# ieellee/uLLSAM

Hardware: AMD Instinct MI355X
Metric: images/s end-to-end (ViT+LLM+mask) 1024^2 (higher is better)
Workload: dtype bf16; 1 GPU; uLLSAM mask path (app.py:580-645): SAM ViT-H + InternLM2-7b-shaped prefill S=1081 + prompt encoder + mask decoder + x4 upsample/threshold, 1 point prompt/image, batch 4/GPU; batch_per_gpu=4, global_batch=4, seq_len=1081, vit_linears=bf16

## Files before the change

### include/ullsam_hip.h

```cpp
#ifndef ULLSAM_HIP_H
#define ULLSAM_HIP_H
#ifdef __cplusplus
extern "C" {
#endif

#define ULLSAM_DT_F32 0
#define ULLSAM_DT_BF16 1
#define ULLSAM_ACT_NONE 0
#define ULLSAM_ACT_GELU 1
#define ULLSAM_ACT_RELU 2
#define ULLSAM_ACT_SWIGLU 3

#define ULLSAM_ABI_VERSION 14

const char* ullsam_last_error_string(void);
int ullsam_abi_version(void);
int ullsam_device_count(void);
int ullsam_set_gemm_variant(int variant);
int ullsam_set_gemm_tuning(int key, int value);
int ullsam_set_attn_variant(int variant);
int ullsam_set_attn_debug(void* stamps);

#define ULLSAM_ACT_SPLITK_OK 256
int ullsam_gemm(int dtype, const void* A, long lda, const void* W, long ldw, void* C, long ldc, int out_f32,
// ... 64 lines not shown
                               void* table_grad, int out_dtype, void* stream);
int ullsam_train_index_add_rows(const float* src, const int* idx, float* dst, long rows, int C, int nrows_dst, void* stream);

int ullsam_norm(const void* in, int in_dtype, long in_stride, void* out, int out_dtype, long out_stride, const float* w,
                const float* b, long rows, int D, float eps, int rms, int act, const float* post_scale,
                const float* post_shift, void* stream);
int ullsam_norm_panels(const void* in, int in_dtype, long in_stride, void* out, const float* w, const float* b, long rows, int D, float eps, int rms,
                       int act, const float* post_scale, const float* post_shift, int out_panels, void* stream);
int ullsam_set_norm_variant(int v);

int ullsam_norm_fanout(const float* in, long rows, int D, const float* w, const float* b, float eps, float* out_f32, void* out_c,
                       void* out_c_pe, int c_dtype, const float* pe, long pe_rows, void* stream);

int ullsam_vit_attention(int dtype, const void* qkv, void* out, const void* rel_h, const void* rel_w, const void* qkv_bias,
                         int B, int heads, int hd, int grid_h, int grid_w, int window, void* stream);

int ullsam_causal_attention(int dtype, const void* q, const void* k, const void* v, void* out, const int* key_mask, int B,
                            int H, int KVH, int hd, int Sq, int Sk, int k_cap, int q_pos0, void* stream);

int ullsam_naive_attention(int dtype, const void* q, const void* k, const void* v, void* out, const int* key_mask, int B,
                           int H, int KVH, int hd, int Sq, int Sk, long q_bs, long q_ts, long q_hs, long k_bs, long k_ts,
                           long k_hs, long v_bs, long v_ts, long v_hs, long o_bs, long o_ts, long o_hs, float scale,
                           void* stream);

int ullsam_decode_attention(const void* q, const void* kc, const void* vc, const int* key_mask, void* out, int B, int H, int KVH,
                            int hd, int Sk, int cap, float scale, float* workspace, int nsplit, void* stream);

int ullsam_fewkeys_attention(const float* q, const float* k, const float* v, float* out, int B, int H, int hd, int Sq,
                             int Sk, float scale, long q_batch_stride, void* stream);

int ullsam_tok2img_attention(int kv_dtype, const float* q, const void* k, const void* v, float* out, int P, int H, int hd, int T,
                             int N, long k_batch_stride, long v_batch_stride, float scale, float* workspace, int nsplit,
                             void* stream);
// ... 223 lines not shown
```

### ullsam_amd/_lib.py

```python
from __future__ import annotations

import ctypes as C
import os

_HERE = os.path.dirname(os.path.abspath(__file__))
LIB_PATH = os.environ.get("ULLSAM_HIP_LIB") or os.path.join(_HERE, "lib", "libullsam_hip.so")

ABI_VERSION = 14

_lib = None

vp, i32, i64, f32 = C.c_void_p, C.c_int, C.c_long, C.c_float

SIGNATURES = {
    "ullsam_gemm": [i32, vp, i64, vp, i64, vp, i64, i32, vp, vp, i64, i32, i32, i32, i32, i32, vp, i64, vp],
    "ullsam_gemm_qkv_rope": [i32, vp, i64, vp, i64, vp, i32, i32, i32, i32, i32, vp, vp, vp, i32, vp, vp, vp, i32, i32, vp, i64, vp],
    "ullsam_gemm_panels": [i32, vp, i64, vp, i64, vp, vp, i64, i32, vp, vp, i64, i32, i32, i32, i32, i32, vp, i64, vp],
    "ullsam_gemm_qkv_rope_panels": [i32, vp, i64, vp, i64, vp, vp, i32, i32, i32, i32, i32, vp, vp, vp, i32, vp, vp, vp, i32, i32, vp, i64, vp],
    "ullsam_gemm_act_panels": [i32, vp, i64, vp, i64, vp, vp, i64, i32, vp, vp, i64, i32, i32, i32, i32, i32, vp, i64, i32, i32, vp],
    "ullsam_gemm_qkv_rope_act_panels": [i32, vp, i64, vp, i64, vp, vp, i32, i32, i32, i32, i32, vp, vp, vp, i32, vp, vp, vp, i32, i32, vp, i64, i32, vp],
    "ullsam_gemm_act_panels_query": [i32, i32, i32, i32, i32, i32, i32, i32, i32, i64, vp, vp],
    "ullsam_gemm_rmsnorm": [vp, i64, vp, f32, vp, i64, vp, i64, i32, vp, vp, i64, i32, i32, i32, i32, vp],
    "ullsam_decode_qkv_rope": [vp, vp, i64, vp, f32, vp, i64, vp, i32, i32, i32, i32, vp, vp, vp, i32, vp, vp, vp, i32, i32, vp],
    "ullsam_train_matmul": [vp, vp, vp, i32, i32, i32, i32] + [i64] * 9 + [i32, vp],
# ... 11 lines not shown
    "ullsam_train_rope": [vp, vp, vp, vp, vp, i64, i32, i32, i32, i32, vp],
    "ullsam_train_swiglu": [vp, vp, vp, vp, vp, vp, i64, vp],
    "ullsam_train_resize_bwd": [vp, vp, i64, i32, i32, i32, i32, vp],
    "ullsam_train_seg_loss": [vp, vp, vp, vp, i32, i64, f32, vp, vp],
    "ullsam_train_seg_loss_bwd": [vp, vp, vp, vp, vp, i32, i64, f32, vp],
    "ullsam_train_cross_entropy": [vp, i64, vp, vp, vp, vp, i64, i32, vp],
    "ullsam_train_cross_entropy_bwd": [vp, i64, vp, vp, vp, vp, vp, i64, i64, i32, vp],
    "ullsam_train_cross_entropy_bwd_bf16": [vp, i64, vp, vp, vp, vp, vp, i64, vp, i64, i64, i32, vp],
    "ullsam_train_embedding_bwd": [vp, i64, vp, vp, vp, i64, i32, i32, i32, vp, i32, vp],
    "ullsam_train_index_add_rows": [vp, vp, vp, i64, i32, i32, vp],
    "ullsam_norm": [vp, i32, i64, vp, i32, i64, vp, vp, i64, i32, f32, i32, i32, vp, vp, vp],
    "ullsam_norm_panels": [vp, i32, i64, vp, vp, vp, i64, i32, f32, i32, i32, vp, vp, i32, vp],
    "ullsam_norm_fanout": [vp, i64, i32, vp, vp, f32, vp, vp, vp, i32, vp, i64, vp],
    "ullsam_vit_attention": [i32, vp, vp, vp, vp, vp, i32, i32, i32, i32, i32, i32, vp],
    "ullsam_causal_attention": [i32, vp, vp, vp, vp, vp, i32, i32, i32, i32, i32, i32, i32, i32, vp],
    "ullsam_naive_attention": [i32, vp, vp, vp, vp, vp, i32, i32, i32, i32, i32, i32] + [i64] * 12 + [f32, vp],
    "ullsam_fewkeys_attention": [vp, vp, vp, vp, i32, i32, i32, i32, i32, f32, i64, vp],
    "ullsam_decode_attention": [vp, vp, vp, vp, vp, i32, i32, i32, i32, i32, i32, f32, vp, i32, vp],
    "ullsam_tok2img_attention": [i32, vp, vp, vp, vp, i32, i32, i32, i32, i32, i64, i64, f32, vp, i32, vp],
    "ullsam_patch_im2col": [i32, vp, vp, i32, i32, i32, i32, i32, i32, vp, vp, vp],
    "ullsam_im2col3x3": [i32, vp, vp, i32, i32, i32, i32, vp],
    "ullsam_add_cast": [vp, i32, i64, vp, i64, vp, i32, i64, i32, vp],
    "ullsam_transpose_f32": [vp, vp, i32, i32, i32, vp],
    "ullsam_transpose_to_bf16": [i32, vp, vp, i32, i32, i32, vp],
    "ullsam_cast_transpose_bf16": [vp, vp, vp, vp, vp, i32, i32, i32, vp],
    "ullsam_pixel_shuffle_ln": [i32, vp, vp, vp, vp, i32, i32, i32, i32, f32, vp],
    "ullsam_pixel_unshuffle": [vp, vp, i32, i32, i32, i32, vp],
    "ullsam_scan_image_tokens": [vp, vp, vp, i32, i32, C.c_longlong, vp],
    "ullsam_embed_tokens": [i32, vp, vp, vp, vp, vp, i32, i32, i32, i32, i64, vp],
    "ullsam_gather_rows": [vp, vp, vp, i32, i32, i32, i32, vp],
# ... 142 lines not shown
```

### ullsam_amd/csrc/attention.hip

```cpp
#include "common.h"
#include <type_traits>

enum { MODE_PLAIN = 0, MODE_CAUSAL = 1, MODE_VIT_GLOBAL = 2, MODE_VIT_WINDOW = 3 };

struct AttnArgs {
    const void* q; const void* k; const void* v; void* out;
    long q_bs, q_ts, q_hs;
    long k_bs, k_ts, k_hs;
    long v_bs, v_ts, v_hs;
    long o_bs, o_ts, o_hs;
    int B, H, groups;
    int Sq, Sk;
    float scale;
    const int* key_mask;
    int q_pos0;
    const void* rel_h; const void* rel_w;
    int grid_h, grid_w;
    int win, nwin_w, nwin;
    const void* bias_q; const void* bias_k; const void* bias_v;
    unsigned long long* dbg;
};

template <typename T, int HD, int TR = 64> struct KVTile {
    static constexpr int RS = HD * (int)sizeof(T) + 16;
    static constexpr int ROWS = TR;
    static constexpr int BYTES = RS * ROWS;
    static constexpr int CPR = HD * (int)sizeof(T) / 16;
    static constexpr int RSV = sizeof(T) == 2 ? 320 : RS;
    static constexpr int VBYTES = RSV * ROWS;
    static_assert(sizeof(T) != 2 || HD * 2 <= 256, "V row does not fit its 320-byte stride");
};

template <int RS>
__device__ __forceinline__ Frag<bf16> load_vt_frag(const char* vt, int kv0, int d0, int lane, const bf16*) {
    const int grp = lane >> 4, i = lane & 15;
    const int h = grp >> 1;
// ... 1002 lines not shown
            mma16(vf[m % NV], pf[m / 5], o[m % 5]);
            if (m % 5 == 4) mma16(ones, pf[m / 5], o[5]);
            __builtin_amdgcn_sched_barrier(0);
            if (m + NV < NVI) vf[m % NV] = vread(m + NV);
        }
        __builtin_amdgcn_sched_barrier(0);
        const float inv_l = 1.0f / o[5][0];
        char* ob = reinterpret_cast<char*>(scr);
#pragma unroll
        for (int d = 0; d < 5; ++d) {
            bf16x4_t v;
            v[0] = (bf16)(o[d][0] * inv_l); v[1] = (bf16)(o[d][1] * inv_l); v[2] = (bf16)(o[d][2] * inv_l); v[3] = (bf16)(o[d][3] * inv_l);
            *reinterpret_cast<bf16x4_t*>(ob + ql * 160 + 32 * d + 8 * g) = v;
        }
        asm volatile("" ::: "memory");
        T* orow = reinterpret_cast<T*>(p.out) + (long)b * p.o_bs + (long)head * p.o_hs;
        const int qgy = wy * G + cur_qh;
#pragma unroll
        for (int r = 0; r < 3; ++r) {
            const int c = lane + 64 * r;
            const int qq = c / 10, ch = c - 10 * qq;
            const int gx = wx * G + qq;
            if (c < 16 * 10 && qq < G && gx < p.grid_w) {
                const uint4 v = *reinterpret_cast<const uint4*>(ob + 16 * c);
                *reinterpret_cast<uint4*>(orow + ((long)qgy * p.grid_w + gx) * p.o_ts + 8 * ch) = v;
            }
        }
        asm volatile("" ::: "memory");
    };
    stamp(2);
    asm volatile("s_waitcnt vmcnt(0)" ::: "memory");
    stamp(3);
    __syncthreads();
    stamp(4);
    if (live[0]) main_group(0, qf0, cinit0, thr0);
    stamp(5);
    if (live[1]) main_group(1, qf1, cinit1, thr1);
    stamp(6);
}

// ... 241 lines not shown
        const unsigned long long s2 = STAMP ? __builtin_amdgcn_s_memtime() : 0ull;
        if (tile + 1 < ntiles && tid < TR) kms[((tile + 1) & 1) * TR + tid] = km_next;
        __syncthreads();
        if (STAMP) { const unsigned long long s3 = __builtin_amdgcn_s_memtime(); st_dma += s1 - s0; st_cmp += s2 - s1; st_bar += s3 - s2; }
    }
    if (STAMP && p.dbg && lane == 0) {
        unsigned long long* d = p.dbg + ((size_t)(blockIdx.y * gridDim.x + blockIdx.x) * 4 + wave) * 8;
        d[0] = st_dma; d[1] = st_cmp; d[2] = st_bar; d[3] = __builtin_amdgcn_s_memtime() - st_t0; d[4] = ntiles; d[5] = qblk;
        d[6] = st_r0; d[7] = __builtin_amdgcn_s_memrealtime();
    }

    float lo, hi;
    halves(l_run, lo, hi);
    const float l_tot = lo + hi;
    const float inv_l = l_tot > 0.f ? 1.0f / l_tot : 0.f;
    if (q_valid) {
        T* op = reinterpret_cast<T*>(p.out) + (long)b * p.o_bs + (long)qi * p.o_ts + (long)head * p.o_hs;
#pragma unroll
        for (int d = 0; d < DT; ++d)
#pragma unroll
            for (int rq = 0; rq < 4; ++rq)
                store4(op + 32 * d + 8 * rq + 4 * h, make_float4(o[d][4 * rq] * inv_l, o[d][4 * rq + 1] * inv_l, o[d][4 * rq + 2] * inv_l, o[d][4 * rq + 3] * inv_l));
    }
}

static int launch_causal128(const AttnArgs& a, hipStream_t s) {
    constexpr int LDS = 2 * 2 * 64 * 256 + 2 * 64 * 4;
    static PerDeviceOnce attr;
    if (attr.first()) {
        (void)hipFuncSetAttribute(reinterpret_cast<const void*>(causal128_attn_kernel<false>), hipFuncAttributeMaxDynamicSharedMemorySize, LDS);
        (void)hipFuncSetAttribute(reinterpret_cast<const void*>(causal128_attn_kernel<true>), hipFuncAttributeMaxDynamicSharedMemorySize, LDS);
    }
    if (a.dbg) causal128_attn_kernel<true><<<dim3(a.H * a.B, (a.Sq + 127) / 128), dim3(256), LDS, s>>>(a);
    else causal128_attn_kernel<false><<<dim3(a.H * a.B, (a.Sq + 127) / 128), dim3(256), LDS, s>>>(a);
    ULLSAM_LAUNCH_CHECK();
    return 0;
}
// ... 239 lines not shown
        };
#pragma unroll 1
        for (int j = 0; j < NB; j += 4) {
            interval(j, I0{}, sc0, sc1);
            interval(j + 1, I1{}, sc1, sc0);
            interval(j + 2, I2{}, sc0, sc1);
            interval(j + 3, I3{}, sc1, sc0);
        }
    }
    asm volatile("s_waitcnt vmcnt(0)" ::: "memory");

    float lo, hi;
    halves(o[DT - 1][8], lo, hi);
    const float l_tot = lo;
    const float inv_l = l_tot > 0.f ? 1.0f / l_tot : 0.f;
    T* op = reinterpret_cast<T*>(p.out) + (long)b * p.o_bs + (long)qi * p.o_ts + (long)head * p.o_hs;
#pragma unroll
    for (int d = 0; d < DT; ++d)
#pragma unroll
        for (int rq = 0; rq < 4; ++rq) {
            const int dd = 32 * d + 8 * rq + 4 * h;
            if (dd < HD) store4(op + dd, make_float4(o[d][4 * rq] * inv_l, o[d][4 * rq + 1] * inv_l, o[d][4 * rq + 2] * inv_l, o[d][4 * rq + 3] * inv_l));
        }
}

static int launch_vitglob(const AttnArgs& a, hipStream_t s) {
    constexpr int LDS = 8 * 32 * 256 + 128 * (80 * 2 + 16) + 8 * 64 * 32 * 4;
    static PerDeviceOnce attr;
    if (attr.first()) (void)hipFuncSetAttribute(reinterpret_cast<const void*>(vitglob_attn_kernel), hipFuncAttributeMaxDynamicSharedMemorySize, LDS);
    vitglob_attn_kernel<<<dim3(a.B * a.H * 16), dim3(512), LDS, s>>>(a);
    ULLSAM_LAUNCH_CHECK();
    return 0;
}

static int g_attn_variant = 0;
static unsigned long long* g_attn_dbg = nullptr;
extern "C" int ullsam_set_attn_variant(int v) { g_attn_variant = v; return 0; }
extern "C" int ullsam_set_attn_debug(void* stamps) { g_attn_dbg = reinterpret_cast<unsigned long long*>(stamps); return 0; }

extern "C" int ullsam_vit_attention(int dtype, const void* qkv, void* out, const void* rel_h, const void* rel_w,
                                    const void* qkv_bias, int B, int heads, int hd, int grid_h, int grid_w, int window,
                                    void* stream) {
    ULLSAM_CHECK(dtype == 0 || dtype == 1, "vit_attention: bad dtype");
    ULLSAM_CHECK(grid_h <= 64 && grid_w <= 64 && window <= 14, "vit_attention: grid %dx%d / window %d too large", grid_h, grid_w, window);
    const int esz = dtype == 0 ? 4 : 2;
    ULLSAM_CHECK((hd * esz) % 16 == 0, "vit_attention: head_dim*elem must be a multiple of 16 bytes");
    ULLSAM_CHECK((((uintptr_t)qkv | (uintptr_t)out | (uintptr_t)qkv_bias | (uintptr_t)rel_h | (uintptr_t)rel_w) & 15) == 0,
                 "vit_attention: qkv, out, rel_h, rel_w and qkv_bias must be 16-byte aligned");
    const long D = (long)heads * hd;
    const long N = (long)grid_h * grid_w;
    AttnArgs a = {};
    const char* base = reinterpret_cast<const char*>(qkv);
    a.q = base; a.k = base + D * esz; a.v = base + 2 * D * esz; a.out = out;
    a.q_bs = a.k_bs = a.v_bs = N * 3 * D; a.q_ts = a.k_ts = a.v_ts = 3 * D; a.q_hs = a.k_hs = a.v_hs = hd;
    a.o_bs = N * D; a.o_ts = D; a.o_hs = hd;
    a.B = B; a.H = heads; a.groups = 1;
    a.scale = 1.0f / sqrtf((float)hd);
    a.rel_h = rel_h; a.rel_w = rel_w; a.grid_h = grid_h; a.grid_w = grid_w;
    const char* bb = reinterpret_cast<const char*>(qkv_bias);
    a.bias_q = bb; a.bias_k = bb + D * esz; a.bias_v = bb + 2 * D * esz;
    hipStream_t s = reinterpret_cast<hipStream_t>(stream);
    if (window > 0) {
        a.win = window;
        a.nwin_w = (grid_w + window - 1) / window;
        a.nwin = a.nwin_w * ((grid_h + window - 1) / window);
        a.Sq = a.Sk = window * window;
        a.q_pos0 = (g_attn_variant >= 3 && g_attn_variant <= 8) ? g_attn_variant - 3 : 2;
        if (dtype == 1 && window == 14 && hd == 80 && g_attn_variant != 1 && g_attn_variant != 2 && g_attn_variant != 13) {
            a.q_pos0 = (g_attn_variant >= 3 && g_attn_variant <= 8) ? g_attn_variant - 3 : 0;
            a.dbg = g_attn_dbg;
            return launch_win14r(a, s);
        }
        if (dtype == 1 && window == 14 && hd == 80 && g_attn_variant != 1 && g_attn_variant != 2) return launch_win14(a, s);
        if (g_attn_variant == 1) return dtype == 0 ? dispatch_hd<float, MODE_VIT_WINDOW, 7>(a, hd, s) : dispatch_hd<bf16, MODE_VIT_WINDOW, 7>(a, hd, s);
        return dtype == 0 ? dispatch_hd<float, MODE_VIT_WINDOW, 7>(a, hd, s) : dispatch_hd<bf16, MODE_VIT_WINDOW, 4>(a, hd, s);
    }
    a.Sq = a.Sk = (int)N;
    if (dtype == 1 && grid_h == 64 && grid_w == 64 && hd == 80 && g_attn_variant != 9 && g_attn_variant != 12)
        return launch_vitglob(a, s);
    if (dtype == 1 && grid_h == 64 && grid_w == 64 && g_attn_variant != 9) return dispatch_hd<bf16, MODE_VIT_GLOBAL, 8>(a, hd, s);
    return dtype == 0 ? dispatch_hd<float, MODE_VIT_GLOBAL, 4>(a, hd, s) : dispatch_hd<bf16, MODE_VIT_GLOBAL, 4>(a, hd, s);
}

extern "C" int ullsam_causal_attention(int dtype, const void* q, const void* k, const void* v, void* out, const int* key_mask,
                                       int B, int H, int KVH, int hd, int Sq, int Sk, int k_cap, int q_pos0, void* stream) {
    ULLSAM_CHECK(dtype == 0 || dtype == 1, "causal_attention: bad dtype");
    ULLSAM_CHECK(H % KVH == 0, "causal_attention: H %% KVH != 0");
    ULLSAM_CHECK((((uintptr_t)q | (uintptr_t)k | (uintptr_t)v | (uintptr_t)out) & 15) == 0, "causal_attention: q, k, v and out must be 16-byte aligned");
    AttnArgs a = {};
    a.q = q; a.k = k; a.v = v; a.out = out;
    a.q_bs = (long)Sq * H * hd; a.q_ts = (long)H * hd; a.q_hs = hd;
    a.k_bs = a.v_bs = (long)KVH * k_cap * hd; a.k_ts = a.v_ts = hd; a.k_hs = a.v_hs = (long)k_cap * hd;
    a.o_bs = a.q_bs; a.o_ts = a.q_ts; a.o_hs = hd;
    a.B = B; a.H = H; a.groups = H / KVH; a.Sq = Sq; a.Sk = Sk; a.key_mask = key_mask; a.q_pos0 = q_pos0;
    a.scale = 1.0f / sqrtf((float)hd);
    a.dbg = g_attn_dbg;
    hipStream_t s = reinterpret_cast<hipStream_t>(stream);
    if (dtype == 1 && hd == 128 && g_attn_variant != 11 && a.k_ts == 128 && a.v_ts == 128)
        return launch_causal128(a, s);
    return dtype == 0 ? dispatch_hd<float, MODE_CAUSAL, 4>(a, hd, s) : dispatch_hd<bf16, MODE_CAUSAL, 4>(a, hd, s);
}

struct NaiveArgs {
    const void* q; const void* k; const void* v; void* out;
    long q_bs, q_ts, q_hs, k_bs, k_ts, k_hs, v_bs, v_ts, v_hs, o_bs, o_ts, o_hs;
    int H, groups, Sq, Sk, hd;
    float scale;
    const int* key_mask;
};

template <typename T>
__global__ __launch_bounds__(256) void naive_attn_kernel(NaiveArgs p) {
    extern __shared__ __attribute__((aligned(16))) char smem[];
    float* sc = reinterpret_cast<float*>(smem);
    float* qs = sc + ((p.Sk + 3) & ~3);
// ... 634 lines not shown
```

### ullsam_amd/modeling/image_encoder.py

```python
from __future__ import annotations

from typing import Optional, Tuple, Type

import torch
from torch import nn

from .. import ops
from ..packing import pack_conv3x3
from .common import LayerNorm, LayerNorm2d, Linear, MLPBlock, Packed


class _Conv2dParams(Packed):

    def __init__(self, cin, cout, k, bias=True):
        super().__init__()
        self.weight = nn.Parameter(torch.empty(cout, cin, k, k))
        self.bias = nn.Parameter(torch.zeros(cout)) if bias else None
        nn.init.normal_(self.weight, std=(cin * k * k) ** -0.5)


class PatchEmbed(Packed):

    def __init__(self, kernel_size=(16, 16), stride=(16, 16), padding=(0, 0), in_chans=3, embed_dim=768):
        super().__init__()
# ... 94 lines not shown
        pos = None if self.pos_embed is None else self.f32("pos", self.pos_embed).reshape(N, D)
        xres = ops.gemm(cols, wp, None if pe.bias is None else self.f32("patch_b", pe.bias), residual=pos, res_row_mod=N, out_f32=True)
        fp8 = bool(self.fp8_linears) and dt == torch.bfloat16 and D % 128 == 0
        M, hp = xres.shape[0], False
        for bi, blk in enumerate(self.blocks):
            at = blk.attn
            if fp8:
                q8, sa = ops.rows_fp8(xres, *blk.norm1.wb(), blk.norm1.eps)
                qkv = ops.gemm_fp8(q8, sa, *at.qkv.w8(), at.qkv.b())
            else:
                ap, _ = ops.activation_panels_plan(M, 3 * D, D, dt, bias=at.qkv.b() is not None)
                xn = ops.norm(xres, *blk.norm1.wb(), blk.norm1.eps, dt, out_panels=ap)
                qkv = ops.gemm(xn, at.qkv.w(dt), at.qkv.b(), w_panels=at.qkv.wp(dt, M), a_panels=ap, m=M)
            qb = at.qkv.bias if at.qkv.bias is not None else torch.zeros(3 * D, device=x.device)
            n_rel = blk.window_size if blk.window_size > 0 else g
            att = ops.vit_attention(qkv, at.rel_table("rh", at.rel_pos_h, n_rel, dt), at.rel_table("rw", at.rel_pos_w, n_rel, dt), at.cdt("qb", qb, dt),
                                    B, self.num_heads, at.head_dim, g, g, blk.window_size)
            ops.gemm(att, at.proj.w(dt), at.proj.b(), residual=xres, out_f32=True, out=xres, w_panels=at.proj.wp(dt, att.shape[0]))
            if fp8:
                q8, sa = ops.rows_fp8(xres, *blk.norm2.wb(), blk.norm2.eps)
                h = ops.gemm_fp8(q8, sa, *blk.mlp.lin1.w8(), blk.mlp.lin1.b(), act=blk.mlp.act_code)
            else:
                w1, w2 = blk.mlp.lin1.w(dt), blk.mlp.lin2.w(dt)
                ap, cp = ops.activation_panels_plan(M, w1.shape[0], D, dt, act=blk.mlp.act_code, bias=blk.mlp.lin1.b() is not None)
                hp = cp and ops.activation_panels_plan(M, D, w2.shape[1], dt, out_f32=True, bias=blk.mlp.lin2.b() is not None, residual=True)[0]
                xn = ops.norm(xres, *blk.norm2.wb(), blk.norm2.eps, dt, out_panels=ap)
                h = ops.gemm(xn, w1, blk.mlp.lin1.b(), act=blk.mlp.act_code, w_panels=blk.mlp.lin1.wp(dt, M), a_panels=ap, out_panels=hp, m=M)
            ops.gemm(h, blk.mlp.lin2.w(dt), blk.mlp.lin2.b(), residual=xres, out_f32=True, out=xres, w_panels=blk.mlp.lin2.wp(dt, M), a_panels=hp, m=M)
            if self.stage_probe is not None:
                self.stage_probe(bi, xres)
        n0, n1, n2, n3 = self.neck[0], self.neck[1], self.neck[2], self.neck[3]
        C = self.out_chans
        w0 = self.pk("neck0", n0.weight, lambda: n0.weight.detach().reshape(C, D).to(dt).contiguous())
# ... 17 lines not shown
```

### ullsam_amd/modeling/modeling_internlm2.py

```python
from __future__ import annotations

from typing import List, Optional, Tuple

import torch
from torch import nn

from .. import ops
from ..packing import pack_w13
from ..sampling import row_seeds
from .common import Linear, Packed, ring_panels
from .configuration_internlm2 import InternLM2Config
from .outputs import BaseModelOutputWithPast, CausalLMOutputWithPast


class InternLM2RMSNorm(Packed):

    def __init__(self, hidden_size, eps=1e-6):
        super().__init__()
        self.weight = nn.Parameter(torch.ones(hidden_size))
        self.variance_epsilon = eps

    def w(self):
        return self.f32("w", self.weight)

# ... 154 lines not shown
            if w8:
                q = ops.decode_qkv_rope_w8(x, layer.attention_norm.w(), layer.attention_norm.variance_epsilon, *at.wqkv.w8d(), at.wqkv.b(), kc, vc,
                                           pos, cos, sin, B, KVH, G, past)
            elif fused:
                q = ops.decode_qkv_rope(x, layer.attention_norm.w(), layer.attention_norm.variance_epsilon, at.wqkv.w(dt), at.wqkv.b(), kc, vc,
                                        pos, cos, sin, B, KVH, G, past)
            else:
                wq, rope_ep = at.wqkv.w(dt), hd == 128 and S > 8
                ap, _ = ops.activation_panels_plan(B * S, wq.shape[0], wq.shape[1], dt, bias=at.wqkv.b() is not None, rope=rope_ep)
                xn = ops.norm(x, layer.attention_norm.w(), None, layer.attention_norm.variance_epsilon, dt, rms=True, out_panels=ap)
                if rope_ep:
                    q = ops.gemm_qkv_rope(xn, wq, at.wqkv.b(), kc, vc, pos, cos, sin, B, S, KVH, G, past, w_panels=at.wqkv.wp(dt, B * S), a_panels=ap)
                else:
                    qkv = ops.gemm(xn, wq, at.wqkv.b(), w_panels=at.wqkv.wp(dt, B * S), a_panels=ap, m=B * S)
                    q = ops.rope_split(qkv, kc, vc, pos, cos, sin, B, S, KVH, G, hd, past)
            if S > 1:
                a = ops.causal_attention(q, kc, vc, key_mask, B, H, KVH, hd, S, Sk, past)
            elif dt == torch.bfloat16 and hd == 128 and G <= 8:
                a = ops.decode_attention(q, kc, vc, key_mask, B, H, KVH, hd, Sk)
            else:
                cap = kc.shape[2]
                a = ops.naive_attention(q, kc, vc, B, H, KVH, hd, 1, Sk, (H * hd, H * hd, hd), (KVH * cap * hd, hd, cap * hd),
                                        (KVH * cap * hd, hd, cap * hd), (H * hd, H * hd, hd), hd ** -0.5, key_mask=key_mask)
            if w8_wo:
                ops.gemm_w8(a, *at.wo.w8d(), at.wo.b(), residual=x, out_f32=True, out=x)
            else:
                ops.gemm(a, at.wo.w(dt), at.wo.b(), residual=x, out_f32=True, out=x, w_panels=at.wo.wp(dt, B * S))
            if w8:
                hmid = ops.gemm_w8(x, *ff.w13_w8d(dt), act=ops.ACT_SWIGLU, norm_w=layer.ffn_norm.w(), eps=layer.ffn_norm.variance_epsilon)
            elif fused:
                hmid = ops.gemm_rmsnorm(x, layer.ffn_norm.w(), layer.ffn_norm.variance_epsilon, ff.w13(dt), act=ops.ACT_SWIGLU)
            else:
                w13, w2 = ff.w13(dt), ff.w2.w(dt)
                ap, cp = ops.activation_panels_plan(B * S, w13.shape[0], w13.shape[1], dt, act=ops.ACT_SWIGLU)
                hp = cp and not w8_w2 and ops.activation_panels_plan(B * S, w2.shape[0], w2.shape[1], dt, out_f32=True, residual=True)[0]
                xn = ops.norm(x, layer.ffn_norm.w(), None, layer.ffn_norm.variance_epsilon, dt, rms=True, out_panels=ap)
                hmid = ops.gemm(xn, w13, act=ops.ACT_SWIGLU, w_panels=ff.w13p(dt, B * S), a_panels=ap, out_panels=hp, m=B * S)
            if w8_w2:
                ops.gemm_w8(hmid, *ff.w2.w8d(), None, residual=x, out_f32=True, out=x)
            else:
                ops.gemm(hmid, ff.w2.w(dt), None, residual=x, out_f32=True, out=x, w_panels=ff.w2.wp(dt, B * S), a_panels=hp, m=B * S)
            if self.stage_probe is not None:
# ... 204 lines not shown
```

### ullsam_amd/ops.py

```python
from __future__ import annotations

import os
from typing import Optional

import numpy as np
import torch

from . import _lib

ACT_NONE, ACT_GELU, ACT_RELU, ACT_SWIGLU = 0, 1, 2, 3
ACT_SPLITK_OK = 256
_DT = {torch.float32: 0, torch.bfloat16: 1}


def dt_code(dtype: torch.dtype) -> int:
    try:
        return _DT[dtype]
    except KeyError:
        raise TypeError(f"ullsam_amd supports float32 and bfloat16 compute, got {dtype}") from None


def _stream() -> int:
    return torch.cuda.current_stream().cuda_stream

# ... 260 lines not shown
    _chk(hs, "hs", torch.float32)
    hyper = torch.empty((P, nm, 32), dtype=torch.float32, device=hs.device)
    iou = torch.empty((P, n_iou), dtype=torch.float32, device=hs.device)
    _lib.call("ullsam_dec_heads", hs.data_ptr(), w_ptrs.data_ptr(), b_ptrs.data_ptr(), hyper.data_ptr(), iou.data_ptr(), P, T, n_iou, m0, nm, _stream())
    return hyper, iou


def concat_token_rows(prefix: torch.Tensor, rows: torch.Tensor) -> torch.Tensor:
    _chk(prefix, "prefix", torch.float32); _chk(rows, "rows", torch.float32)
    P, n1, C = rows.shape
    out = torch.empty((P, prefix.shape[0] + n1, C), dtype=torch.float32, device=rows.device)
    _lib.call("ullsam_concat_token_rows", prefix.data_ptr(), prefix.shape[0], rows.data_ptr() if n1 else None, n1, out.data_ptr(), P, C, _stream())
    return out


def vit_attention(qkv: torch.Tensor, rel_h: torch.Tensor, rel_w: torch.Tensor, qkv_bias: torch.Tensor, B: int, heads: int,
                  hd: int, gh: int, gw: int, window: int) -> torch.Tensor:
    _chk(qkv, "qkv"); _chk(rel_h, "rel_h", qkv.dtype); _chk(rel_w, "rel_w", qkv.dtype); _chk(qkv_bias, "qkv_bias", qkv.dtype)
    D = heads * hd
    assert qkv.numel() == B * gh * gw * 3 * D
    n = window if window > 0 else gh
    assert rel_h.shape == (2 * n - 1, hd) and rel_w.shape[1] == hd
    out = torch.empty((B * gh * gw, D), dtype=qkv.dtype, device=qkv.device)
    _lib.call("ullsam_vit_attention", dt_code(qkv.dtype), qkv.data_ptr(), out.data_ptr(), rel_h.data_ptr(), rel_w.data_ptr(),
              qkv_bias.data_ptr(), B, heads, hd, gh, gw, window, _stream())
    return out


def causal_attention(q: torch.Tensor, k_cache: torch.Tensor, v_cache: torch.Tensor, key_mask: Optional[torch.Tensor],
                     B: int, H: int, KVH: int, hd: int, Sq: int, Sk: int, q_pos0: int) -> torch.Tensor:
    _chk(q, "q"); _chk(k_cache, "k_cache", q.dtype); _chk(v_cache, "v_cache", q.dtype)
    cap = k_cache.shape[2]
    if key_mask is not None:
        _chk(key_mask, "key_mask", torch.int32)
        assert key_mask.shape == (B, Sk)
    out = torch.empty((B * Sq, H * hd), dtype=q.dtype, device=q.device)
    _lib.call("ullsam_causal_attention", dt_code(q.dtype), q.data_ptr(), k_cache.data_ptr(), v_cache.data_ptr(), out.data_ptr(),
              _p(key_mask), B, H, KVH, hd, Sq, Sk, cap, q_pos0, _stream())
    return out


def naive_attention(q, k, v, B, H, KVH, hd, Sq, Sk, qs, ks, vs, os_, scale, key_mask=None, out=None):
    _chk(q, "q"); _chk(k, "k", q.dtype); _chk(v, "v", q.dtype)
    if out is None:
        out = torch.empty((B * Sq, H * hd), dtype=q.dtype, device=q.device)
    if key_mask is not None:
        _chk(key_mask, "key_mask", torch.int32)
    _lib.call("ullsam_naive_attention", dt_code(q.dtype), q.data_ptr(), k.data_ptr(), v.data_ptr(), out.data_ptr(), _p(key_mask),
              B, H, KVH, hd, Sq, Sk, *qs, *ks, *vs, *os_, float(scale), _stream())
    return out

# ... 1797 lines not shown
```

Baseline: 58.07 images/s.

## Write attention outputs directly in GEMM K-panel layout for output projections

The ViT windowed/global attention and the LLM causal prefill attention kernels can now stage their output tile in LDS and store it in the 16x32 K-panel layout that the following output-projection GEMM consumes as pre-paneled A. The proj/wo GEMMs are then called with a_panels set, so they skip their own repacking of the activation. Query entry points report whether the chosen kernel supports this, and an environment mask turns it on by default. The cost is extra LDS staging and swizzled scatter stores in the attention epilogues, plus a 1 KiB alignment requirement on the output buffer.

```diff
diff --git a/include/ullsam_hip.h b/include/ullsam_hip.h
--- a/include/ullsam_hip.h
+++ b/include/ullsam_hip.h
@@ -102,9 +102,15 @@
 
 int ullsam_vit_attention(int dtype, const void* qkv, void* out, const void* rel_h, const void* rel_w, const void* qkv_bias,
                          int B, int heads, int hd, int grid_h, int grid_w, int window, void* stream);
+int ullsam_vit_attention_out(int dtype, const void* qkv, void* out, const void* rel_h, const void* rel_w, const void* qkv_bias,
+                             int B, int heads, int hd, int grid_h, int grid_w, int window, int out_panels, void* stream);
+int ullsam_vit_attention_panels_query(int dtype, int heads, int hd, int grid_h, int grid_w, int window, int* writes_panels);
 
 int ullsam_causal_attention(int dtype, const void* q, const void* k, const void* v, void* out, const int* key_mask, int B,
                             int H, int KVH, int hd, int Sq, int Sk, int k_cap, int q_pos0, void* stream);
+int ullsam_causal_attention_out(int dtype, const void* q, const void* k, const void* v, void* out, const int* key_mask, int B,
+                                int H, int KVH, int hd, int Sq, int Sk, int k_cap, int q_pos0, int out_mode, void* stream);
+int ullsam_causal_attention_panels_query(int dtype, int H, int KVH, int hd, int* writes_panels);
 
 int ullsam_naive_attention(int dtype, const void* q, const void* k, const void* v, void* out, const int* key_mask, int B,
                            int H, int KVH, int hd, int Sq, int Sk, long q_bs, long q_ts, long q_hs, long k_bs, long k_ts,
diff --git a/ullsam_amd/_lib.py b/ullsam_amd/_lib.py
--- a/ullsam_amd/_lib.py
+++ b/ullsam_amd/_lib.py
@@ -49,6 +49,10 @@
     "ullsam_norm_fanout": [vp, i64, i32, vp, vp, f32, vp, vp, vp, i32, vp, i64, vp],
     "ullsam_vit_attention": [i32, vp, vp, vp, vp, vp, i32, i32, i32, i32, i32, i32, vp],
     "ullsam_causal_attention": [i32, vp, vp, vp, vp, vp, i32, i32, i32, i32, i32, i32, i32, i32, vp],
+    "ullsam_vit_attention_out": [i32, vp, vp, vp, vp, vp, i32, i32, i32, i32, i32, i32, i32, vp],
+    "ullsam_vit_attention_panels_query": [i32, i32, i32, i32, i32, i32, vp],
+    "ullsam_causal_attention_out": [i32, vp, vp, vp, vp, vp, i32, i32, i32, i32, i32, i32, i32, i32, i32, vp],
+    "ullsam_causal_attention_panels_query": [i32, i32, i32, i32, vp],
     "ullsam_naive_attention": [i32, vp, vp, vp, vp, vp, i32, i32, i32, i32, i32, i32] + [i64] * 12 + [f32, vp],
     "ullsam_fewkeys_attention": [vp, vp, vp, vp, i32, i32, i32, i32, i32, f32, i64, vp],
     "ullsam_decode_attention": [vp, vp, vp, vp, vp, i32, i32, i32, i32, i32, i32, f32, vp, i32, vp],
diff --git a/ullsam_amd/csrc/attention.hip b/ullsam_amd/csrc/attention.hip
--- a/ullsam_amd/csrc/attention.hip
+++ b/ullsam_amd/csrc/attention.hip
@@ -19,7 +19,13 @@
     int win, nwin_w, nwin;
     const void* bias_q; const void* bias_k; const void* bias_v;
     unsigned long long* dbg;
+    int out_mode;
 };
+enum { ATTN_OUT_ROWS = 0, ATTN_OUT_ROWS_STAGED = 1, ATTN_OUT_PANELS = 2 };
+
+__device__ __forceinline__ long panel_at(long row, int col, int K) {
+    return ((row >> 4) * (K >> 5) + (col >> 5)) * 512 + (row & 15) * 32 + (col & 31);
+}
 
 template <typename T, int HD, int TR = 64> struct KVTile {
     static constexpr int RS = HD * (int)sizeof(T) + 16;
@@ -1052,7 +1058,9 @@
             *reinterpret_cast<bf16x4_t*>(ob + ql * 160 + 32 * d + 8 * g) = v;
         }
         asm volatile("" ::: "memory");
-        T* orow = reinterpret_cast<T*>(p.out) + (long)b * p.o_bs + (long)head * p.o_hs;
+        const bool panels = p.out_mode == ATTN_OUT_PANELS;
+        T* orow = reinterpret_cast<T*>(p.out) + (panels ? 0 : (long)b * p.o_bs + (long)head * p.o_hs);
+        const long prow0 = (long)b * p.grid_h * p.grid_w;
         const int qgy = wy * G + cur_qh;
 #pragma unroll
         for (int r = 0; r < 3; ++r) {
@@ -1061,7 +1069,8 @@
             const int gx = wx * G + qq;
             if (c < 16 * 10 && qq < G && gx < p.grid_w) {
                 const uint4 v = *reinterpret_cast<const uint4*>(ob + 16 * c);
-                *reinterpret_cast<uint4*>(orow + ((long)qgy * p.grid_w + gx) * p.o_ts + 8 * ch) = v;
+                const long tok = (long)qgy * p.grid_w + gx;
+                *reinterpret_cast<uint4*>(orow + (panels ? panel_at(prow0 + tok, head * 80 + 8 * ch, (int)p.o_ts) : tok * p.o_ts + 8 * ch)) = v;
             }
         }
         asm volatile("" ::: "memory");
@@ -1333,13 +1342,40 @@
     halves(l_run, lo, hi);
     const float l_tot = lo + hi;
     const float inv_l = l_tot > 0.f ? 1.0f / l_tot : 0.f;
-    if (q_valid) {
-        T* op = reinterpret_cast<T*>(p.out) + (long)b * p.o_bs + (long)qi * p.o_ts + (long)head * p.o_hs;
-#pragma unroll
-        for (int d = 0; d < DT; ++d)
-#pragma unroll
-            for (int rq = 0; rq < 4; ++rq)
-                store4(op + 32 * d + 8 * rq + 4 * h, make_float4(o[d][4 * rq] * inv_l, o[d][4 * rq + 1] * inv_l, o[d][4 * rq + 2] * inv_l, o[d][4 * rq + 3] * inv_l));
+    if (p.out_mode == ATTN_OUT_ROWS) {
+        if (q_valid) {
+            T* op = reinterpret_cast<T*>(p.out) + (long)b * p.o_bs + (long)qi * p.o_ts + (long)head * p.o_hs;
+#pragma unroll
+            for (int d = 0; d < DT; ++d)
+#pragma unroll
+                for (int rq = 0; rq < 4; ++rq)
+                    store4(op + 32 * d + 8 * rq + 4 * h, make_float4(o[d][4 * rq] * inv_l, o[d][4 * rq + 1] * inv_l, o[d][4 * rq + 2] * inv_l, o[d][4 * rq + 3] * inv_l));
+        }
+        return;
+    }
+    char* img = smem + wave * 8192;
+#pragma unroll
+    for (int d = 0; d < DT; ++d)
+#pragma unroll
+        for (int rq = 0; rq < 4; ++rq) {
+            bf16x4_t v;
+            v[0] = (bf16)(o[d][4 * rq] * inv_l); v[1] = (bf16)(o[d][4 * rq + 1] * inv_l); v[2] = (bf16)(o[d][4 * rq + 2] * inv_l); v[3] = (bf16)(o[d][4 * rq + 3] * inv_l);
+            *reinterpret_cast<bf16x4_t*>(img + 256 * ql + 16 * ((4 * d + rq) ^ swq) + 8 * h) = v;
+        }
+    asm volatile("" ::: "memory");
+    const bool panels = p.out_mode == ATTN_OUT_PANELS;
+    const int row0 = qbase + wave * 32, Kdim = (int)p.o_ts;
+    T* const ob = reinterpret_cast<T*>(p.out);
+#pragma unroll
+    for (int i = 0; i < 8; ++i) {
+        const int r = panels ? 16 * (i >> 2) + (lane >> 2) : 4 * i + (lane >> 4);
+        const int c = panels ? 4 * (i & 3) + (lane & 3) : lane & 15;
+        const int qr = row0 + r;
+        if (qr >= 0 && qr < p.Sq) {
+            const uint4 v = *reinterpret_cast<const uint4*>(img + 256 * r + 16 * (c ^ (((r & 3) << 2) | ((r >> 2) & 3))));
+            const long at = panels ? panel_at((long)b * p.Sq + qr, head * HD + 8 * c, Kdim) : (long)b * p.o_bs + (long)qr * p.o_ts + (long)head * p.o_hs + 8 * c;
+            *reinterpret_cast<uint4*>(ob + at) = v;
+        }
     }
 }
 
@@ -1609,14 +1645,47 @@
     halves(o[DT - 1][8], lo, hi);
     const float l_tot = lo;
     const float inv_l = l_tot > 0.f ? 1.0f / l_tot : 0.f;
-    T* op = reinterpret_cast<T*>(p.out) + (long)b * p.o_bs + (long)qi * p.o_ts + (long)head * p.o_hs;
+    if (p.out_mode != ATTN_OUT_PANELS) {
+        T* op = reinterpret_cast<T*>(p.out) + (long)b * p.o_bs + (long)qi * p.o_ts + (long)head * p.o_hs;
+#pragma unroll
+        for (int d = 0; d < DT; ++d)
+#pragma unroll
+            for (int rq = 0; rq < 4; ++rq) {
+                const int dd = 32 * d + 8 * rq + 4 * h;
+                if (dd < HD) store4(op + dd, make_float4(o[d][4 * rq] * inv_l, o[d][4 * rq + 1] * inv_l, o[d][4 * rq + 2] * inv_l, o[d][4 * rq + 3] * inv_l));
+            }
+        return;
+    }
+    char* img = smem + RELH + wave * 8192;
 #pragma unroll
     for (int d = 0; d < DT; ++d)
 #pragma unroll
         for (int rq = 0; rq < 4; ++rq) {
-            const int dd = 32 * d + 8 * rq + 4 * h;
-            if (dd < HD) store4(op + dd, make_float4(o[d][4 * rq] * inv_l, o[d][4 * rq + 1] * inv_l, o[d][4 * rq + 2] * inv_l, o[d][4 * rq + 3] * inv_l));
-        }
+            if (32 * d + 8 * rq < HD) {
+                bf16x4_t v;
+                v[0] = (bf16)(o[d][4 * rq] * inv_l); v[1] = (bf16)(o[d][4 * rq + 1] * inv_l); v[2] = (bf16)(o[d][4 * rq + 2] * inv_l); v[3] = (bf16)(o[d][4 * rq + 3] * inv_l);
+                *reinterpret_cast<bf16x4_t*>(img + 256 * ql + 16 * ((4 * d + rq) ^ swq) + 8 * h) = v;
+            }
+        }
+    asm volatile("" ::: "memory");
+    const int odd = head & 1;
+    const long row0 = (long)b * p.Sq + qblk * 256 + wave * 32;
+    T* const ob = reinterpret_cast<T*>(p.out);
+#pragma unroll
+    for (int i = 0; i < 5; ++i) {
+        const int e = 64 * i + lane, rb = e >= 160, f = e - 160 * rb;
+        int row, ch;
+        if (odd) {
+            if (f < 32) { row = f >> 1; ch = f & 1; }
+            else { const int g = f - 32; row = (g & 63) >> 2; ch = 2 + 4 * (g >> 6) + (g & 3); }
+        } else {
+            if (f < 128) { row = (f & 63) >> 2; ch = 4 * (f >> 6) + (f & 3); }
+            else { row = (f - 128) >> 1; ch = 8 + (f & 1); }
+        }
+        const int r = 16 * rb + row;
+        const uint4 v = *reinterpret_cast<const uint4*>(img + 256 * r + 16 * (ch ^ (((r & 3) << 2) | ((r >> 2) & 3))));
+        *reinterpret_cast<uint4*>(ob + panel_at(row0 + r, head * HD + 8 * ch, (int)p.o_ts)) = v;
+    }
 }
 
 static int launch_vitglob(const AttnArgs& a, hipStream_t s) {
@@ -1633,9 +1702,9 @@
 extern "C" int ullsam_set_attn_variant(int v) { g_attn_variant = v; return 0; }
 extern "C" int ullsam_set_attn_debug(void* stamps) { g_attn_dbg = reinterpret_cast<unsigned long long*>(stamps); return 0; }
 
-extern "C" int ullsam_vit_attention(int dtype, const void* qkv, void* out, const void* rel_h, const void* rel_w,
-                                    const void* qkv_bias, int B, int heads, int hd, int grid_h, int grid_w, int window,
-                                    void* stream) {
+static int vit_attention_impl(int dtype, const void* qkv, void* out, const void* rel_h, const void* rel_w,
+                              const void* qkv_bias, int B, int heads, int hd, int grid_h, int grid_w, int window,
+                              void* stream, int out_panels, int* plan) {
     ULLSAM_CHECK(dtype == 0 || dtype == 1, "vit_attention: bad dtype");
     ULLSAM_CHECK(grid_h <= 64 && grid_w <= 64 && window <= 14, "vit_attention: grid %dx%d / window %d too large", grid_h, grid_w, window);
     const int esz = dtype == 0 ? 4 : 2;
@@ -1664,21 +1733,57 @@
         if (dtype == 1 && window == 14 && hd == 80 && g_attn_variant != 1 && g_attn_variant != 2 && g_attn_variant != 13) {
             a.q_pos0 = (g_attn_variant >= 3 && g_attn_variant <= 8) ? g_attn_variant - 3 : 0;
             a.dbg = g_attn_dbg;
+            const bool p_ok = D % 32 == 0;
+            if (plan) { *plan = p_ok; return 0; }
+            if (out_panels) {
+                ULLSAM_CHECK(p_ok && ((uintptr_t)out & 1023) == 0, "vit_attention: panel output needs heads * hd %% 32 == 0 and a 1 KiB aligned buffer");
+                a.out_mode = ATTN_OUT_PANELS;
+            }
             return launch_win14r(a, s);
         }
+        if (plan) { *plan = 0; return 0; }
+        ULLSAM_CHECK(!out_panels, "vit_attention: this launch does not reach the kernel that writes K-panels -- ask ullsam_vit_attention_panels_query first");
         if (dtype == 1 && window == 14 && hd == 80 && g_attn_variant != 1 && g_attn_variant != 2) return launch_win14(a, s);
         if (g_attn_variant == 1) return dtype == 0 ? dispatch_hd<float, MODE_VIT_WINDOW, 7>(a, hd, s) : dispatch_hd<bf16, MODE_VIT_WINDOW, 7>(a, hd, s);
         return dtype == 0 ? dispatch_hd<float, MODE_VIT_WINDOW, 7>(a, hd, s) : dispatch_hd<bf16, MODE_VIT_WINDOW, 4>(a, hd, s);
     }
     a.Sq = a.Sk = (int)N;
-    if (dtype == 1 && grid_h == 64 && grid_w == 64 && hd == 80 && g_attn_variant != 9 && g_attn_variant != 12)
+    if (dtype == 1 && grid_h == 64 && grid_w == 64 && hd == 80 && g_attn_variant != 9 && g_attn_variant != 12) {
+        const bool p_ok = D % 32 == 0;
+        if (plan) { *plan = p_ok; return 0; }
+        if (out_panels) {
+            ULLSAM_CHECK(p_ok && ((uintptr_t)out & 1023) == 0, "vit_attention: panel output needs heads * hd %% 32 == 0 and a 1 KiB aligned buffer");
+            a.out_mode = ATTN_OUT_PANELS;
+        }
         return launch_vitglob(a, s);
+    }
+    if (plan) { *plan = 0; return 0; }
+    ULLSAM_CHECK(!out_panels, "vit_attention: this launch does not reach a kernel that writes K-panels -- ask ullsam_vit_attention_panels_query first");
     if (dtype == 1 && grid_h == 64 && grid_w == 64 && g_attn_variant != 9) return dispatch_hd<bf16, MODE_VIT_GLOBAL, 8>(a, hd, s);
     return dtype == 0 ? dispatch_hd<float, MODE_VIT_GLOBAL, 4>(a, hd, s) : dispatch_hd<bf16, MODE_VIT_GLOBAL, 4>(a, hd, s);
 }
 
-extern "C" int ullsam_causal_attention(int dtype, const void* q, const void* k, const void* v, void* out, const int* key_mask,
-                                       int B, int H, int KVH, int hd, int Sq, int Sk, int k_cap, int q_pos0, void* stream) {
+extern "C" int ullsam_vit_attention(int dtype, const void* qkv, void* out, const void* rel_h, const void* rel_w,
+                                    const void* qkv_bias, int B, int heads, int hd, int grid_h, int grid_w, int window,
+                                    void* stream) {
+    return vit_attention_impl(dtype, qkv, out, rel_h, rel_w, qkv_bias, B, heads, hd, grid_h, grid_w, window, stream, 0, nullptr);
+}
+
+extern "C" int ullsam_vit_attention_out(int dtype, const void* qkv, void* out, const void* rel_h, const void* rel_w,
+                                        const void* qkv_bias, int B, int heads, int hd, int grid_h, int grid_w, int window,
+                                        int out_panels, void* stream) {
+    return vit_attention_impl(dtype, qkv, out, rel_h, rel_w, qkv_bias, B, heads, hd, grid_h, grid_w, window, stream, out_panels != 0, nullptr);
+}
+
+extern "C" int ullsam_vit_attention_panels_query(int dtype, int heads, int hd, int grid_h, int grid_w, int window, int* writes_panels) {
+    ULLSAM_CHECK(writes_panels, "ullsam_vit_attention_panels_query: null answer");
+    *writes_panels = 0;
+    alignas(16) static const char dummy[16] = {};
+    return vit_attention_impl(dtype, dummy, const_cast<char*>(dummy), dummy, dummy, dummy, 1, heads, hd, grid_h, grid_w, window, nullptr, 0, writes_panels);
+}
+
+static int causal_attention_impl(int dtype, const void* q, const void* k, const void* v, void* out, const int* key_mask,
+                                 int B, int H, int KVH, int hd, int Sq, int Sk, int k_cap, int q_pos0, void* stream, int out_mode, int* plan) {
     ULLSAM_CHECK(dtype == 0 || dtype == 1, "causal_attention: bad dtype");
     ULLSAM_CHECK(H % KVH == 0, "causal_attention: H %% KVH != 0");
     ULLSAM_CHECK((((uintptr_t)q | (uintptr_t)k | (uintptr_t)v | (uintptr_t)out) & 15) == 0, "causal_attention: q, k, v and out must be 16-byte aligned");
@@ -1691,9 +1796,33 @@
     a.scale = 1.0f / sqrtf((float)hd);
     a.dbg = g_attn_dbg;
     hipStream_t s = reinterpret_cast<hipStream_t>(stream);
-    if (dtype == 1 && hd == 128 && g_attn_variant != 11 && a.k_ts == 128 && a.v_ts == 128)
+    if (dtype == 1 && hd == 128 && g_attn_variant != 11 && a.k_ts == 128 && a.v_ts == 128) {
+        if (plan) { *plan = 1; return 0; }
+        ULLSAM_CHECK(out_mode != ATTN_OUT_PANELS || ((uintptr_t)out & 1023) == 0, "causal_attention: the panel output needs a 1 KiB aligned buffer");
+        a.out_mode = out_mode;
         return launch_causal128(a, s);
+    }
+    if (plan) { *plan = 0; return 0; }
+    ULLSAM_CHECK(out_mode == ATTN_OUT_ROWS, "causal_attention: this launch does not reach the kernel that stages its stores -- ask ullsam_causal_attention_panels_query first");
     return dtype == 0 ? dispatch_hd<float, MODE_CAUSAL, 4>(a, hd, s) : dispatch_hd<bf16, MODE_CAUSAL, 4>(a, hd, s);
+}
+
+extern "C" int ullsam_causal_attention(int dtype, const void* q, const void* k, const void* v, void* out, const int* key_mask,
+                                       int B, int H, int KVH, int hd, int Sq, int Sk, int k_cap, int q_pos0, void* stream) {
+    return causal_attention_impl(dtype, q, k, v, out, key_mask, B, H, KVH, hd, Sq, Sk, k_cap, q_pos0, stream, ATTN_OUT_ROWS, nullptr);
+}
+
+extern "C" int ullsam_causal_attention_out(int dtype, const void* q, const void* k, const void* v, void* out, const int* key_mask,
+                                           int B, int H, int KVH, int hd, int Sq, int Sk, int k_cap, int q_pos0, int out_mode, void* stream) {
+    ULLSAM_CHECK(out_mode >= 0 && out_mode <= 2, "causal_attention_out: out_mode %d", out_mode);
+    return causal_attention_impl(dtype, q, k, v, out, key_mask, B, H, KVH, hd, Sq, Sk, k_cap, q_pos0, stream, out_mode, nullptr);
+}
+
+extern "C" int ullsam_causal_attention_panels_query(int dtype, int H, int KVH, int hd, int* writes_panels) {
+    ULLSAM_CHECK(writes_panels, "ullsam_causal_attention_panels_query: null answer");
+    *writes_panels = 0;
+    alignas(16) static const char dummy[16] = {};
+    return causal_attention_impl(dtype, dummy, dummy, dummy, const_cast<char*>(dummy), nullptr, 1, H, KVH, hd, 1, 1, 1, 0, nullptr, ATTN_OUT_ROWS, writes_panels);
 }
 
 struct NaiveArgs {
diff --git a/ullsam_amd/modeling/image_encoder.py b/ullsam_amd/modeling/image_encoder.py
--- a/ullsam_amd/modeling/image_encoder.py
+++ b/ullsam_amd/modeling/image_encoder.py
@@ -132,9 +132,11 @@
                 qkv = ops.gemm(xn, at.qkv.w(dt), at.qkv.b(), w_panels=at.qkv.wp(dt, M), a_panels=ap, m=M)
             qb = at.qkv.bias if at.qkv.bias is not None else torch.zeros(3 * D, device=x.device)
             n_rel = blk.window_size if blk.window_size > 0 else g
+            pp = (ops.activation_panels_plan(M, D, D, dt, out_f32=True, bias=at.proj.b() is not None, residual=True)[0]
+                  and ops.vit_attention_panels_ok(dt, self.num_heads, at.head_dim, g, g, blk.window_size))
             att = ops.vit_attention(qkv, at.rel_table("rh", at.rel_pos_h, n_rel, dt), at.rel_table("rw", at.rel_pos_w, n_rel, dt), at.cdt("qb", qb, dt),
-                                    B, self.num_heads, at.head_dim, g, g, blk.window_size)
-            ops.gemm(att, at.proj.w(dt), at.proj.b(), residual=xres, out_f32=True, out=xres, w_panels=at.proj.wp(dt, att.shape[0]))
+                                    B, self.num_heads, at.head_dim, g, g, blk.window_size, out_panels=pp)
+            ops.gemm(att, at.proj.w(dt), at.proj.b(), residual=xres, out_f32=True, out=xres, w_panels=at.proj.wp(dt, M), a_panels=pp, m=M)
             if fp8:
                 q8, sa = ops.rows_fp8(xres, *blk.norm2.wb(), blk.norm2.eps)
                 h = ops.gemm_fp8(q8, sa, *blk.mlp.lin1.w8(), blk.mlp.lin1.b(), act=blk.mlp.act_code)
diff --git a/ullsam_amd/modeling/modeling_internlm2.py b/ullsam_amd/modeling/modeling_internlm2.py
--- a/ullsam_amd/modeling/modeling_internlm2.py
+++ b/ullsam_amd/modeling/modeling_internlm2.py
@@ -192,8 +192,12 @@
                 else:
                     qkv = ops.gemm(xn, wq, at.wqkv.b(), w_panels=at.wqkv.wp(dt, B * S), a_panels=ap, m=B * S)
                     q = ops.rope_split(qkv, kc, vc, pos, cos, sin, B, S, KVH, G, hd, past)
+            wo_ap = False
             if S > 1:
-                a = ops.causal_attention(q, kc, vc, key_mask, B, H, KVH, hd, S, Sk, past)
+                wo = at.wo.w(dt)
+                wo_ap = (ops.activation_panels_plan(B * S, wo.shape[0], wo.shape[1], dt, out_f32=True, bias=at.wo.b() is not None, residual=True)[0]
+                         and ops.causal_attention_panels_ok(dt, H, KVH, hd))
+                a = ops.causal_attention(q, kc, vc, key_mask, B, H, KVH, hd, S, Sk, past, out_mode=ops.CAUSAL_OUT_PANELS if wo_ap else ops.CAUSAL_OUT_ROWS)
             elif dt == torch.bfloat16 and hd == 128 and G <= 8:
                 a = ops.decode_attention(q, kc, vc, key_mask, B, H, KVH, hd, Sk)
             else:
@@ -203,7 +207,7 @@
             if w8_wo:
                 ops.gemm_w8(a, *at.wo.w8d(), at.wo.b(), residual=x, out_f32=True, out=x)
             else:
-                ops.gemm(a, at.wo.w(dt), at.wo.b(), residual=x, out_f32=True, out=x, w_panels=at.wo.wp(dt, B * S))
+                ops.gemm(a, at.wo.w(dt), at.wo.b(), residual=x, out_f32=True, out=x, w_panels=at.wo.wp(dt, B * S), a_panels=wo_ap, m=B * S)
             if w8:
                 hmid = ops.gemm_w8(x, *ff.w13_w8d(dt), act=ops.ACT_SWIGLU, norm_w=layer.ffn_norm.w(), eps=layer.ffn_norm.variance_epsilon)
             elif fused:
diff --git a/ullsam_amd/ops.py b/ullsam_amd/ops.py
--- a/ullsam_amd/ops.py
+++ b/ullsam_amd/ops.py
@@ -298,27 +298,80 @@
     return out
 
 
+_ATTN_PANELS = int(os.environ.get("ULLSAM_ATTENTION_PANELS", "3")) & 3
+
+
+def set_attention_panels(mask: int) -> None:
+    global _ATTN_PANELS
+    _ATTN_PANELS = int(mask) & 3
+
+
+def vit_attention_panels_ok(dtype: torch.dtype, heads: int, hd: int, gh: int, gw: int, window: int) -> bool:
+    if not _ATTN_PANELS & 2:
+        return False
+    import ctypes
+    ans = ctypes.c_int(0)
+    _lib.call("ullsam_vit_attention_panels_query", dt_code(dtype), heads, hd, gh, gw, window, ctypes.addressof(ans))
+    return bool(ans.value)
+
+
 def vit_attention(qkv: torch.Tensor, rel_h: torch.Tensor, rel_w: torch.Tensor, qkv_bias: torch.Tensor, B: int, heads: int,
-                  hd: int, gh: int, gw: int, window: int) -> torch.Tensor:
+                  hd: int, gh: int, gw: int, window: int, out_panels: bool = False, out: Optional[torch.Tensor] = None) -> torch.Tensor:
     _chk(qkv, "qkv"); _chk(rel_h, "rel_h", qkv.dtype); _chk(rel_w, "rel_w", qkv.dtype); _chk(qkv_bias, "qkv_bias", qkv.dtype)
     D = heads * hd
     assert qkv.numel() == B * gh * gw * 3 * D
     n = window if window > 0 else gh
     assert rel_h.shape == (2 * n - 1, hd) and rel_w.shape[1] == hd
-    out = torch.empty((B * gh * gw, D), dtype=qkv.dtype, device=qkv.device)
+    if out_panels:
+        if out is None:
+            out = empty_activation_panels(B * gh * gw, D, qkv.device)
+        _chk(out, "out", qkv.dtype)
+        assert out.shape == ((B * gh * gw + 15) // 16 * 16, D)
+        _lib.call("ullsam_vit_attention_out", dt_code(qkv.dtype), qkv.data_ptr(), out.data_ptr(), rel_h.data_ptr(), rel_w.data_ptr(),
+                  qkv_bias.data_ptr(), B, heads, hd, gh, gw, window, 1, _stream())
+        return out
+    if out is None:
+        out = torch.empty((B * gh * gw, D), dtype=qkv.dtype, device=qkv.device)
+    _chk(out, "out", qkv.dtype)
+    assert out.shape == (B * gh * gw, D)
     _lib.call("ullsam_vit_attention", dt_code(qkv.dtype), qkv.data_ptr(), out.data_ptr(), rel_h.data_ptr(), rel_w.data_ptr(),
               qkv_bias.data_ptr(), B, heads, hd, gh, gw, window, _stream())
     return out
 
 
+CAUSAL_OUT_ROWS, CAUSAL_OUT_ROWS_STAGED, CAUSAL_OUT_PANELS = 0, 1, 2
+
+
+def causal_attention_panels_ok(dtype: torch.dtype, H: int, KVH: int, hd: int) -> bool:
+    if not _ATTN_PANELS & 1:
+        return False
+    import ctypes
+    ans = ctypes.c_int(0)
+    _lib.call("ullsam_causal_attention_panels_query", dt_code(dtype), H, KVH, hd, ctypes.addressof(ans))
+    return bool(ans.value)
+
+
 def causal_attention(q: torch.Tensor, k_cache: torch.Tensor, v_cache: torch.Tensor, key_mask: Optional[torch.Tensor],
-                     B: int, H: int, KVH: int, hd: int, Sq: int, Sk: int, q_pos0: int) -> torch.Tensor:
+                     B: int, H: int, KVH: int, hd: int, Sq: int, Sk: int, q_pos0: int, out_mode: int = CAUSAL_OUT_ROWS,
+                     out: Optional[torch.Tensor] = None) -> torch.Tensor:
     _chk(q, "q"); _chk(k_cache, "k_cache", q.dtype); _chk(v_cache, "v_cache", q.dtype)
     cap = k_cache.shape[2]
     if key_mask is not None:
         _chk(key_mask, "key_mask", torch.int32)
         assert key_mask.shape == (B, Sk)
-    out = torch.empty((B * Sq, H * hd), dtype=q.dtype, device=q.device)
+    if out_mode != CAUSAL_OUT_ROWS:
+        rows = (B * Sq + 15) // 16 * 16 if out_mode == CAUSAL_OUT_PANELS else B * Sq
+        if out is None:
+            out = empty_activation_panels(B * Sq, H * hd, q.device) if out_mode == CAUSAL_OUT_PANELS else torch.empty((rows, H * hd), dtype=q.dtype, device=q.device)
+        _chk(out, "out", q.dtype)
+        assert out.shape == (rows, H * hd)
+        _lib.call("ullsam_causal_attention_out", dt_code(q.dtype), q.data_ptr(), k_cache.data_ptr(), v_cache.data_ptr(), out.data_ptr(),
+                  _p(key_mask), B, H, KVH, hd, Sq, Sk, cap, q_pos0, out_mode, _stream())
+        return out
+    if out is None:
+        out = torch.empty((B * Sq, H * hd), dtype=q.dtype, device=q.device)
+    _chk(out, "out", q.dtype)
+    assert out.shape == (B * Sq, H * hd)
     _lib.call("ullsam_causal_attention", dt_code(q.dtype), q.data_ptr(), k_cache.data_ptr(), v_cache.data_ptr(), out.data_ptr(),
               _p(key_mask), B, H, KVH, hd, Sq, Sk, cap, q_pos0, _stream())
     return out
```

Result: no change. 58.31 images/s (median of 6 runs) (+0.4%).
